# tianhao-stan-wu/LLA-MPC

Hardware: AMD Instinct MI355X
Metric: model-rollouts/sec (N_models x H steps) per control tick; wall-clock per plan() call (higher is better)
Workload: dtype f64

## Files before the change

lla-mpc_amd/csrc/dev_wave.hpp:

```cpp
#pragma once
#include <hip/hip_runtime.h>
#include <stdint.h>

#include "kernels.hpp"

namespace llampc {

namespace {

template <int NAN_FIRST>
__device__ __forceinline__ bool kless(double av, int64_t ai, double bv, int64_t bi) {
  return NAN_FIRST ? less_nan_first(av, ai, bv, bi) : less_nan_last(av, ai, bv, bi);
}

constexpr int kDppXor1 = 0xB1, kDppXor2 = 0x4E, kDppRor4 = 0x124, kDppRor8 = 0x128;
template <int CTRL>
__device__ __forceinline__ int dpp_i(int x) {
  return __builtin_amdgcn_update_dpp(x, x, CTRL, 0xF, 0xF, false);
}
template <int CTRL>
__device__ __forceinline__ double dpp_d(double v) {
  return __hiloint2double(dpp_i<CTRL>(__double2hiint(v)), dpp_i<CTRL>(__double2loint(v)));
}
template <int CTRL>
// ... 119 lines not shown
__device__ __forceinline__ uint64_t join_words(uint64_t hi, uint64_t lo) {
  return ((uint64_t)(uint32_t)hi << 32) | (uint32_t)lo;
}

__device__ __forceinline__ int wave_sum(int x) {
  x += dpp_i<kDppXor1>(x);
  x += dpp_i<kDppXor2>(x);
  x += dpp_i<kDppRor4>(x);
  x += dpp_i<kDppRor8>(x);
  return __builtin_amdgcn_readlane(x, 0) + __builtin_amdgcn_readlane(x, 16) +
         __builtin_amdgcn_readlane(x, 32) + __builtin_amdgcn_readlane(x, 48);
}

__device__ __forceinline__ void pin_vgpr(double& x) { asm volatile("" : "+v"(x)); }

}

constexpr int kScratchBytes = 192;
constexpr int kFlagOff = 160;
constexpr int kLateOff = 168;
constexpr int kStageW = 8;
constexpr int kRankBytes = 64 * 8 + 64 * 4 + 256;
constexpr int kWaves = kBlock / 64;
constexpr int kListsPerLane = 8;

struct Scratch {
  double* sv;
  int64_t* si;
  int32_t* sn;
  __device__ explicit Scratch(unsigned char* smem)
// ... 40 lines not shown
```

lla-mpc_amd/csrc/kernels.hip:

```cpp
#include <stdlib.h>

#include <algorithm>

#include "dev_wave.hpp"
#include "final_dev.hpp"
#include "lookback_dev.hpp"
#include "peer_dev.hpp"
#include "rollout_dev.hpp"

namespace llampc {

__global__ __launch_bounds__(kBlock) void merge_kernel(const llampc_plan_out* parts, int32_t G,
                                                       int32_t nan_first, llampc_plan_out* m) {
  extern __shared__ __attribute__((aligned(16))) unsigned char smem[];
  const int tid = threadIdx.x;
  llampc_plan_out* rec = reinterpret_cast<llampc_plan_out*>(smem);
  constexpr int kWords = sizeof(llampc_plan_out) / 16;
  static_assert(sizeof(llampc_plan_out) % 16 == 0, "records staged as 16-B words");
  const uint4* srcw = reinterpret_cast<const uint4*>(parts);
  uint4* dstw = reinterpret_cast<uint4*>(rec);
  for (int e = tid; e < G * kWords; e += kBlock) dstw[e] = srcw[e];
  __syncthreads();
  merge_staged(rec, G, nan_first, m, reinterpret_cast<EntS*>(smem + (size_t)G * sizeof(llampc_plan_out)), 0);
}
// ... 225 lines not shown
      if (base + rl > kLdsMax) {
        stage = false;
        base = kScratchBytes + 16 * (size_t)(la->H + 1);
      }
      const size_t per_seg = 32 * (size_t)std::max(1, la->rl.M);
      const size_t room = base + rl < kLdsMax ? kLdsMax - base - rl : 0;
      lav.rl.wcap = (int32_t)std::min<size_t>(room / per_seg, (size_t)(la->rl.n - 1));
      lds = std::max(lds, base + rl + per_seg * (size_t)lav.rl.wcap);
    } else {
      lds = std::max(lds, lookahead_lds_bytes(la->C, la->H, &stage));
    }
  }
  f.do_lb = lb != nullptr;
  f.do_la = la != nullptr;
  if (f.nb_lb + f.nb_la == 0) return hipErrorInvalidValue;
  int wq = 0;
  if (la && la->wq && lpm == 1 && G <= 64 && integ == LLAMPC_RK4 && la->xref_mode == LLAMPC_XREF_GIVEN &&
      !pk && getenv("LLAMPC_NO_WQ") == nullptr) {
    const int nw = std::max(1, device_cus() - 1);
    const char* force = getenv("LLAMPC_WQ_WAVES");
    const int forced = force ? atoi(force) : 0;
    if ((int64_t)f.nb_la * 4 >= (int64_t)nw * 7 || (forced && f.nb_la > nw)) {
      const int64_t mpw = 64 / G;
      const int64_t units = (la->n + mpw - 1) / mpw;
      f.nb_la = nw;
      wq = (stage && (forced ? forced == 8 : units >= 4 * (int64_t)nw * kWaves)) ? 2 : 1;
    }
  }
  if (f.px_G) {
    if (pk || integ != LLAMPC_RK4 || (la && la->xref_mode == LLAMPC_XREF_RACELINE) || f.px_G > kPeerFuseMax)
      return hipErrorInvalidValue;
    lds = std::max(lds, 256 + (size_t)f.px_G * (sizeof(llampc_plan_out) + 2 * LLAMPC_KMAX * sizeof(EntS)) +
                            kWaves * sizeof(int));
  }

  if (pk) {
    if (!la || !plan_inline_ok(la->C, la->H, integ, la->xref_mode) || !stage) return hipErrorInvalidValue;
    if (lpm == 4) launch_plan_inline_group<4>(lbv, lav, f, G, cpl, lds, s, *pk);
    else if (lpm == 2) launch_plan_inline_group<2>(lbv, lav, f, G, cpl, lds, s, *pk);
    else launch_plan_inline_group<1>(lbv, lav, f, G, cpl, lds, s, *pk);
    return hipGetLastError();
  }
  switch (integ) {
    case LLAMPC_RK4:
    case LLAMPC_EULER_NLP: {
      const bool rk4 = integ == LLAMPC_RK4;
      const int w = rk4 ? wq : 0;
      if (lpm == 4) (rk4 ? launch_plan_group<0, 4> : launch_plan_group<1, 4>)(lbv, lav, f, G, cpl, stage, lds, s, w);
      else if (lpm == 2) (rk4 ? launch_plan_group<0, 2> : launch_plan_group<1, 2>)(lbv, lav, f, G, cpl, stage, lds, s, w);
      else (rk4 ? launch_plan_group<0, 1> : launch_plan_group<1, 1>)(lbv, lav, f, G, cpl, stage, lds, s, w);
      break;
    }
    case LLAMPC_RK6:
      launch_plan_group<2, 1>(lbv, lav, f, G, cpl, stage, lds, s, 0);
      break;
    default: return hipErrorInvalidValue;
  }
  return hipGetLastError();
}


hipError_t launch_merge(const llampc_plan_out* parts, int32_t G, int32_t nan_first,
                        llampc_plan_out* merged, hipStream_t s) {
  if (G < 1 || G > 32) return hipErrorInvalidValue;
  const size_t M = (size_t)G * LLAMPC_KMAX;
  const size_t lds = (size_t)G * sizeof(llampc_plan_out) + 2 * M * sizeof(EntS);
  allow_lds(merge_kernel);
  hipLaunchKernelGGL(merge_kernel, dim3(1), dim3(kBlock), lds, s, parts, G, nan_first, merged);
  return hipGetLastError();
// ... 46 lines not shown
```

lla-mpc_amd/csrc/kernels.hpp:

```cpp
#pragma once
#include <hip/hip_runtime.h>
#include <stdint.h>

#include "dyn.hpp"
#include "raceline.hpp"
#include "llampc.h"

namespace llampc {

constexpr int kBlock = 256;
constexpr int kBlockWQ = 512;
constexpr int wq_threads(int wq) { return wq == 2 ? kBlockWQ : kBlock; }

struct CostK {
  double Q[4], R[4], P[4];
  double umin[2], umax[2];
  double dmax[2];
  int32_t enforce;
  int32_t pad;
};

struct LookbackLaunch {
  const double* params;  int64_t n;  int64_t goff;
  VehK veh;
// ... 40 lines not shown
  const double* am_val; const int64_t* am_idx; const double* tk_val; const int64_t* tk_idx;
  const double* pv; const int64_t* pidx; const int32_t* pnf;
  const uint64_t* la_tag; const uint64_t* blk_tag;
  uint32_t seq;
  int32_t poll;
  uint64_t* host_tag;
  uint64_t host_seq;
  uint64_t* const* px_box;
  llampc_plan_out* px_merged;
  int32_t px_G, px_rank;
  uint32_t px_seq;
  uint32_t px_bound;
  uint64_t* wq;
};

constexpr int kInlineDoubles = 352;
struct InlinePack {
  double v[kInlineDoubles];
};

int lookback_blocks(int64_t n);
int lookahead_group(int32_t C);
int lookahead_lpm(int64_t n, int32_t C, int32_t integrator, int32_t share = 1);
int lookahead_blocks(int64_t n, int32_t C, int lpm);
int lookback_r(int64_t n, int32_t K);
int lookback_blocks_r(int64_t n, int R);
size_t lookahead_lds_bytes(int32_t C, int32_t H, bool* stage_u);
size_t raceline_lds_bytes(int32_t n, int32_t M);

hipError_t launch_plan(const LookbackLaunch* lb, const LookaheadLaunch* la, FinalLaunch f,
                       hipStream_t s, const InlinePack* pk = nullptr, int32_t share = 1);
bool plan_inline_ok(int32_t C, int32_t H, int32_t integrator, int32_t xref_mode);
template <int INTEG, int LPM>
void launch_plan_group(const LookbackLaunch& lb, const LookaheadLaunch& la, const FinalLaunch& f, int G,
                       int cpl, bool stage, size_t lds, hipStream_t s, int wq);
template <int LPM>
void launch_plan_inline_group(const LookbackLaunch& lb, const LookaheadLaunch& la, const FinalLaunch& f,
                              int G, int cpl, size_t lds, hipStream_t s, const InlinePack& pk);
#define LLAMPC_PLAN_GROUP_DECL(I, L)                                                               \
  extern template void launch_plan_group<I, L>(const LookbackLaunch&, const LookaheadLaunch&,      \
                                               const FinalLaunch&, int, int, bool, size_t,          \
                                               hipStream_t, int)
LLAMPC_PLAN_GROUP_DECL(0, 4);
LLAMPC_PLAN_GROUP_DECL(0, 2);
LLAMPC_PLAN_GROUP_DECL(0, 1);
LLAMPC_PLAN_GROUP_DECL(1, 4);
LLAMPC_PLAN_GROUP_DECL(1, 2);
LLAMPC_PLAN_GROUP_DECL(1, 1);
LLAMPC_PLAN_GROUP_DECL(2, 1);
extern template void launch_plan_inline_group<4>(const LookbackLaunch&, const LookaheadLaunch&, const FinalLaunch&,
                                                 int, int, size_t, hipStream_t, const InlinePack&);
extern template void launch_plan_inline_group<2>(const LookbackLaunch&, const LookaheadLaunch&, const FinalLaunch&,
                                                 int, int, size_t, hipStream_t, const InlinePack&);
extern template void launch_plan_inline_group<1>(const LookbackLaunch&, const LookaheadLaunch&, const FinalLaunch&,
                                                 int, int, size_t, hipStream_t, const InlinePack&);
template <typename KERN>
static void allow_lds(KERN k) {
  static bool done = false;
  if (!done) {
    (void)hipFuncSetAttribute(reinterpret_cast<const void*>(k), hipFuncAttributeMaxDynamicSharedMemorySize,
                              (int)(160 * 1024));
    done = true;
  }
}
hipError_t launch_merge(const llampc_plan_out* parts, int32_t G, int32_t nan_first,
                        llampc_plan_out* merged, hipStream_t s);
constexpr int kPeerMax = 32;
constexpr int kRecWords = (int)(sizeof(llampc_plan_out) / 4);
struct PeerLaunch {
  const llampc_plan_out* local;
// ... 19 lines not shown
```

lla-mpc_amd/csrc/lookahead_dev.hpp:

```cpp
#pragma once
#include "dev_stamps.hpp"
#include "dev_wave.hpp"
#include "raceline.hpp"
#include "rollout_dev.hpp"

namespace llampc {

template <int NW = kWaves>
__device__ __forceinline__ void la_publish(const LookaheadLaunch& a, int blk, const Scratch& sc, int par,
                                           double v, int64_t key, int nf) {
  static_assert(NW == kWaves || NW == 8, "4- or 8-wave blocks");
  wave_pick_nl64(v, key);
  const int nfw = wave_sum(nf);
  double* sv = sc.sv + 4 * par;
  int64_t* si = sc.si + 4 * par;
  if ((threadIdx.x & 63) == 0) {
    sv[threadIdx.x >> 6] = v;
    si[threadIdx.x >> 6] = key;
    sc.sn[threadIdx.x >> 6] = nfw;
  }
  __syncthreads();
  if (threadIdx.x == 0) {
    int nfs = sc.sn[0];
#pragma unroll
// ... 7 lines not shown
      uint64_t* r = a.blk_tag + 5 * (int64_t)blk;
      const uint64_t vb = (uint64_t)__double_as_longlong(v), kb = (uint64_t)key;
      st_wt(&r[0], tag_word(a.seq, (uint32_t)(vb >> 32)));
      st_wt(&r[1], tag_word(a.seq, (uint32_t)vb));
      st_wt(&r[2], tag_word(a.seq, (uint32_t)(kb >> 32)));
      st_wt(&r[3], tag_word(a.seq, (uint32_t)kb));
      st_wt(&r[4], tag_word(a.seq, (uint32_t)nfs));
    } else {
      st_wt(&a.pv[blk], v);
      st_wt(&a.pidx[blk], key);
      st_wt(&a.pnf[blk], nfs);
    }
  }
}

template <int INTEG, bool STAGE, int LPM, int XM, int WQ = 0>
__device__ __forceinline__ void lookahead_block(const LookaheadLaunch& a, int blk, int G, int cpl,
                                                unsigned char* smem, const Scratch& sc) {
  LA_STAMP(blk, 0);
  constexpr int BT = wq_threads(WQ);
  double* sx = reinterpret_cast<double*>(smem + kScratchBytes);
  double* su = sx + 2 * (a.H + 1);
  const int H = a.H, C = a.C;
  const int sub = threadIdx.x % LPM;
  const int cl = threadIdx.x / LPM;
  const int g = cl & (G - 1);
  const int64_t n = (int64_t)blk * (kBlock / (G * LPM)) + cl / G;
  const bool live = n < a.n;
  const int mpb = kBlock / (G * LPM);
  const int soff = (XM && mpb < kBlock) ? mpb : 0;
  Tire t{};
  if (!WQ && live) t = load_tire(a.params, a.n, n);
  double x0[6];
#pragma unroll
  for (int m = 0; m < 6; ++m) x0[m] = a.x0[m];
  double* rl_knots = su + (STAGE ? kStageW * C * H : 0);
  double* rl_xy = rl_knots + a.rl.n + kKnotPad;
  if (XM) {
    const int nk = a.rl.n, nseg = a.rl.n - 1, nxy = 8 * nseg;
    const double* gk = a.rl.knots;
    const double* gmu = a.rl.mus;
    double* rl_mus = rl_xy + nxy;
    copy_lds<4>(rl_knots, nk, [&](int e) { return gk[e]; });
    copy_lds<24>(rl_xy, nxy + a.rl.M, [&](int e) {
      const double* p = e < nxy ? gk + nk + e : gmu + (e - nxy);
      return *p;
    });
    if ((int)threadIdx.x < kKnotPad) rl_knots[nk + threadIdx.x] = __builtin_inf();
    const double s0 = a.xref[0];
    const double L = gk[nseg];
// ... 69 lines not shown
    RL_STAMP(blk, 3);
  } else {
    for (int e = threadIdx.x; e <= H; e += BT) {
      sx[2 * e] = a.xref[e];
      sx[2 * e + 1] = a.xref[(H + 1) + e];
    }
  }
  fm::FmK K0;
  if constexpr (!XM) K0 = fm::FmK::load<kLeanLA && INTEG == 0>();
  if (STAGE) {
    const fm::FmK K = [&] {
      if constexpr (XM) return fm::FmK::load();
      else return K0;
    }();
    const FusedK fq0 = make_fused(a.veh, make_stage<1>(a.veh, Tire{}, 0), a.Ts, scaled_yaw(LPM));
    for (int e = (int)threadIdx.x - soff; e < C * H; e += BT - soff) {
      if (e < 0) break;
      const int c = e / H, k = e - c * H;
      const double dl = a.U[2 * e + 1];
      double sd, cd;
      if (fm::sincos_fast_ok(dl)) fm::sincos_fast(dl, &sd, &cd, K);
      else LL_SINCOS(dl, &sd, &cd);
      double* o = su + kStageW * (k * C + c);
      const double ua = a.U[2 * e];
      const double p0 = k ? a.U[2 * e - 2] : a.uprev[0], p1 = k ? a.U[2 * e - 1] : a.uprev[1];
      const double d0 = ua - p0, d1 = dl - p1;
      if (INTEG == 0) {
        const FusedIn fi = fused_in(fq0, Input{ua, dl, sd, cd});
        o[0] = fi.F0;
        o[1] = fi.F1;
        o[2] = fi.hmsd;
        o[3] = fi.hmcd;
        o[4] = fi.c5a;
        o[5] = dl;
      } else {
        o[0] = ua;
        o[1] = dl;
        o[2] = sd;
        o[3] = cd;
      }
      o[6] = act_term(a.cost, d0, d1);
      o[7] = (!a.cost.enforce || input_feasible(a.cost, ua, dl, d0, d1)) ? 1.0 : 0.0;
    }
  }
  __syncthreads();

  CostK q = a.cost;
  VehK veh = a.veh;
  double Ts = a.Ts;
  for (int m = 0; m < 4; ++m) {
    pin_vgpr(q.Q[m]);
    pin_vgpr(q.R[m]);
    pin_vgpr(q.P[m]);
  }
  for (int m = 0; m < 2; ++m) {
    pin_vgpr(q.umin[m]);
    pin_vgpr(q.umax[m]);
    pin_vgpr(q.dmax[m]);
  }
  pin_vgpr(veh.lf);
  pin_vgpr(veh.lr);
  pin_vgpr(veh.mass);
  pin_vgpr(veh.inv_mass);
  pin_vgpr(veh.inv_Iz);
  pin_vgpr(veh.Cm1);
  pin_vgpr(veh.Cm2);
  pin_vgpr(veh.Cr0);
  pin_vgpr(veh.Cr2);
  pin_vgpr(Ts);
  const double up0 = a.uprev[0], up1 = a.uprev[1];

  double bv = __builtin_nan("");
  int64_t bc = kNoIndex;
  int nf = 0;
  LA_STAMP(blk, 1);
  constexpr bool kSplit = (INTEG == 0 && LPM == 4);
  constexpr unsigned kRF = (STAGE ? kRStage : 0u) | (XM ? kRXm : 0u);
  constexpr unsigned kRSplitQ = kSplit ? kRSplit : 0u;
  const bool diagQP = a.cost.Q[1] == 0.0 && a.cost.Q[2] == 0.0 && a.cost.P[1] == 0.0 && a.cost.P[2] == 0.0;
  if constexpr (WQ) {
    static_assert(LPM == 1 && XM == 0, "work queue: LPM 1, shared xref");
    const int mpw = 64 / G;
    const int64_t units = (a.n + mpw - 1) / mpw;
    const int lm = (int)(threadIdx.x & 63) / G;
    uint32_t zoff;
    asm volatile("v_mov_b32 %0, 0" : "=v"(zoff));
    auto issue = [&](uint32_t off) -> uint64_t {
      uint64_t v = 0;
      if ((threadIdx.x & 63) == 0)
        v = __hip_atomic_fetch_add(a.wq + off, (uint64_t)1, __ATOMIC_RELAXED, __HIP_MEMORY_SCOPE_AGENT);
      return v;
    };
    auto take = [&](uint64_t v) -> int64_t {
      const uint32_t lo = (uint32_t)__builtin_amdgcn_readlane((int)(uint32_t)v, 0);
// ... 184 lines not shown
```

lla-mpc_amd/csrc/plan_dev.hpp:

```cpp
#pragma once
#include <algorithm>

#include "final_dev.hpp"
#include "lookahead_dev.hpp"
#include "lookback_dev.hpp"
#include "peer_dev.hpp"

namespace llampc {

template <int INTEG, bool STAGE, int LPM, int XM, bool PX = false, int WQ = 0>
__device__ __forceinline__ void plan_body(const LookbackLaunch& lb, const LookaheadLaunch& la,
                                          const FinalLaunch& fin, int G, int cpl) {
  extern __shared__ __attribute__((aligned(16))) unsigned char smem[];
  const Scratch sc(smem);
  int* flag = reinterpret_cast<int*>(smem + kFlagOff);
  const bool is_lb = (int)blockIdx.x < fin.nb_lb;
  const int lb_blk = (int)blockIdx.x, la_blk = (int)blockIdx.x - fin.nb_lb;
  if constexpr (wq_threads(WQ) > kBlock) {
    if (is_lb && threadIdx.x >= kBlock) return;
  }
  if (is_lb) {
    lookback_block(lb, lb_blk, sc);
    if (!ticket_last(&fin.tickets[0], (unsigned)fin.nb_lb, flag)) return;
    if (fin.full) {
      lb_final(fin, smem);
      if (fin.host_tag) __threadfence_system();
    }
    if (fin.poll) {
      __syncthreads();
      final_poll(fin, sc);
      if constexpr (PX) peer_finish(fin, smem);
      return;
    }
  } else {
    lookahead_block<INTEG, STAGE, LPM, XM, WQ>(la, la_blk, G, cpl, smem, sc);
    if (fin.poll) return;
    if constexpr (wq_threads(WQ) > kBlock) {
      if (threadIdx.x >= kBlock) return;
    }
  }
  const unsigned expected = (unsigned)fin.nb_la + (fin.nb_lb > 0 ? 1u : 0u);
  if (!ticket_last(&fin.tickets[1], expected, flag)) return;
  final_select(fin, sc);
  if constexpr (PX) peer_finish(fin, smem);
}

template <int INTEG, bool STAGE, int LPM, int XM, bool PX = false, int WQ = 0>
__global__ __launch_bounds__(wq_threads(WQ)) void plan_kernel(LookbackLaunch lb, LookaheadLaunch la,
                                                      FinalLaunch fin, int G, int cpl) {
  plan_body<INTEG, STAGE, LPM, XM, PX, WQ>(lb, la, fin, G, cpl);
}

template <int LPM>
__global__ __launch_bounds__(kBlock) void plan_kernel_inl(LookbackLaunch lb, LookaheadLaunch la,
                                                          FinalLaunch fin, int G, int cpl,
                                                          InlinePack pk) {
  const double* v = pk.v;
  lb.x_prev = v;
  lb.u_prev = v + 6;
  lb.x_now = v + 8;
  la.x0 = v + 8;
  la.uprev = v + 14;
  la.xref = v + 16;
  la.U = v + 16 + 2 * (la.H + 1);
  plan_body<0, true, LPM, 0>(lb, la, fin, G, cpl);
}

constexpr size_t kOneBlockPerCuLds = 82 * 1024;

template <int INTEG, bool STAGE, int PX, int WQ>
static void launch_plan_wq(const LookbackLaunch& lb, const LookaheadLaunch& la, const FinalLaunch& f,
                           int G, int cpl, size_t lds, hipStream_t s) {
  allow_lds(plan_kernel<INTEG, STAGE, 1, 0, PX, WQ>);
  hipLaunchKernelGGL((plan_kernel<INTEG, STAGE, 1, 0, PX, WQ>), dim3(f.nb_lb + f.nb_la), dim3(wq_threads(WQ)),
                     lds, s, lb, la, f, G, cpl);
}

template <int INTEG, bool STAGE, int LPM>
static void launch_plan_t(const LookbackLaunch& lb, const LookaheadLaunch& la, const FinalLaunch& f,
                          int G, int cpl, size_t lds, hipStream_t s, int wq = 0) {
  lds = std::max(lds, kOneBlockPerCuLds);
  if constexpr (INTEG == LLAMPC_RK4 && LPM == 1) {
    if (wq) {
      if constexpr (STAGE) {
        if (wq == 2) {
          if (f.px_G) launch_plan_wq<INTEG, STAGE, 1, 2>(lb, la, f, G, cpl, lds, s);
          else launch_plan_wq<INTEG, STAGE, 0, 2>(lb, la, f, G, cpl, lds, s);
          return;
        }
      }
      if (f.px_G) launch_plan_wq<INTEG, STAGE, 1, 1>(lb, la, f, G, cpl, lds, s);
      else launch_plan_wq<INTEG, STAGE, 0, 1>(lb, la, f, G, cpl, lds, s);
      return;
    }
  }
  if constexpr (INTEG == LLAMPC_RK4) {
    if (f.px_G) {
      allow_lds(plan_kernel<INTEG, STAGE, LPM, 0, true>);
      hipLaunchKernelGGL((plan_kernel<INTEG, STAGE, LPM, 0, true>), dim3(f.nb_lb + f.nb_la), dim3(kBlock), lds,
                         s, lb, la, f, G, cpl);
      return;
    }
  }
  if (la.xref_mode == LLAMPC_XREF_RACELINE) {
    allow_lds(plan_kernel<INTEG, STAGE, LPM, 1>);
    hipLaunchKernelGGL((plan_kernel<INTEG, STAGE, LPM, 1>), dim3(f.nb_lb + f.nb_la), dim3(kBlock), lds, s,
                       lb, la, f, G, cpl);
  } else {
    allow_lds(plan_kernel<INTEG, STAGE, LPM, 0>);
    hipLaunchKernelGGL((plan_kernel<INTEG, STAGE, LPM, 0>), dim3(f.nb_lb + f.nb_la), dim3(kBlock), lds, s,
                       lb, la, f, G, cpl);
  }
}

template <int LPM>
static void launch_plan_inl(const LookbackLaunch& lb, const LookaheadLaunch& la, const FinalLaunch& f,
                            int G, int cpl, size_t lds, hipStream_t s, const InlinePack& pk) {
  lds = std::max(lds, kOneBlockPerCuLds);
  allow_lds(plan_kernel_inl<LPM>);
  hipLaunchKernelGGL((plan_kernel_inl<LPM>), dim3(f.nb_lb + f.nb_la), dim3(kBlock), lds, s, lb, la, f,
                     G, cpl, pk);
}

template <int INTEG, int LPM>
void launch_plan_group(const LookbackLaunch& lb, const LookaheadLaunch& la, const FinalLaunch& f, int G,
                       int cpl, bool stage, size_t lds, hipStream_t s, int wq) {
  if (stage) launch_plan_t<INTEG, true, LPM>(lb, la, f, G, cpl, lds, s, wq);
  else launch_plan_t<INTEG, false, LPM>(lb, la, f, G, cpl, lds, s, wq);
}

template <int LPM>
void launch_plan_inline_group(const LookbackLaunch& lb, const LookaheadLaunch& la, const FinalLaunch& f,
                              int G, int cpl, size_t lds, hipStream_t s, const InlinePack& pk) {
  launch_plan_inl<LPM>(lb, la, f, G, cpl, lds, s, pk);
}

}
```

lla-mpc_amd/csrc/plan_euler.hip:

```cpp
#include "plan_dev.hpp"

namespace llampc {

template void launch_plan_group<1, 4>(const LookbackLaunch&, const LookaheadLaunch&, const FinalLaunch&, int,
                                            int, bool, size_t, hipStream_t, int);
template void launch_plan_group<1, 2>(const LookbackLaunch&, const LookaheadLaunch&, const FinalLaunch&, int,
                                            int, bool, size_t, hipStream_t, int);
template void launch_plan_group<1, 1>(const LookbackLaunch&, const LookaheadLaunch&, const FinalLaunch&, int,
                                            int, bool, size_t, hipStream_t, int);

}
```

lla-mpc_amd/csrc/plan_rk4_l1.hip:

```cpp
#include "plan_dev.hpp"

namespace llampc {

template void launch_plan_group<0, 1>(const LookbackLaunch&, const LookaheadLaunch&, const FinalLaunch&, int,
                                            int, bool, size_t, hipStream_t, int);
template void launch_plan_inline_group<1>(const LookbackLaunch&, const LookaheadLaunch&, const FinalLaunch&,
                                              int, int, size_t, hipStream_t, const InlinePack&);

}

#ifdef LLAMPC_STAMPS
namespace llampc {
extern "C" int llampc_debug_wq_units(unsigned long long* out) {
  return hipMemcpyFromSymbol(out, HIP_SYMBOL(g_wq_unit), sizeof(g_wq_unit)) == hipSuccess ? 0 : -2;
}
extern "C" int llampc_debug_wq_reset() {
  void* p = nullptr;
  if (hipGetSymbolAddress(&p, HIP_SYMBOL(g_wq_unit)) != hipSuccess) return -2;
  return hipMemset(p, 0, sizeof(g_wq_unit)) == hipSuccess ? 0 : -2;
}
}
#endif
```

lla-mpc_amd/csrc/plan_rk4_l2.hip:

```cpp
#include "plan_dev.hpp"

namespace llampc {

template void launch_plan_group<0, 2>(const LookbackLaunch&, const LookaheadLaunch&, const FinalLaunch&, int,
                                            int, bool, size_t, hipStream_t, int);
template void launch_plan_inline_group<2>(const LookbackLaunch&, const LookaheadLaunch&, const FinalLaunch&,
                                              int, int, size_t, hipStream_t, const InlinePack&);

}
```

lla-mpc_amd/csrc/plan_rk4_l4.hip:

```cpp
#include "plan_dev.hpp"

namespace llampc {

template void launch_plan_group<0, 4>(const LookbackLaunch&, const LookaheadLaunch&, const FinalLaunch&, int,
                                            int, bool, size_t, hipStream_t, int);
template void launch_plan_inline_group<4>(const LookbackLaunch&, const LookaheadLaunch&, const FinalLaunch&,
                                              int, int, size_t, hipStream_t, const InlinePack&);

}

#ifdef LLAMPC_STAMPS
namespace llampc {
extern "C" int llampc_debug_lb_stamps(unsigned long long* out) {
  return hipMemcpyFromSymbol(out, HIP_SYMBOL(g_lb_stamps), sizeof(g_lb_stamps)) == hipSuccess ? 0 : -2;
}
extern "C" int llampc_debug_rl_ph(unsigned long long* out) {
  return hipMemcpyFromSymbol(out, HIP_SYMBOL(g_rl_ph), sizeof(g_rl_ph)) == hipSuccess ? 0 : -2;
}
extern "C" int llampc_debug_rl(double* out) {
  return hipMemcpyFromSymbol(out, HIP_SYMBOL(g_rl_dbg), sizeof(g_rl_dbg)) == hipSuccess ? 0 : -2;
}
extern "C" int llampc_debug_la_wave(unsigned long long* out) {
  return hipMemcpyFromSymbol(out, HIP_SYMBOL(g_la_wave), sizeof(g_la_wave)) == hipSuccess ? 0 : -2;
}
// ... 16 lines not shown
```

lla-mpc_amd/csrc/plan_rk6.hip:

```cpp
#include "plan_dev.hpp"

namespace llampc {

template void launch_plan_group<2, 1>(const LookbackLaunch&, const LookaheadLaunch&, const FinalLaunch&, int,
                                            int, bool, size_t, hipStream_t, int);

}
```

Before: 8.347 billion.

## Pack plan kernel arguments into a single head-first kernarg struct with scalar pinning

Replaces the separate lookback/lookahead/final launch structs with one PlanArgs kernarg block. Its leading PlanHead holds the hot shared fields within a few adjacent cache lines, and the role structs are read in 16-byte words. Device code reads fields through kernarg-segment pointers, pins pointers and scalars into SGPRs via readfirstlane and address-space casts, and hoists the initial U/uprev/x0 loads so they overlap LDS staging. The aim is to cut kernel-argument fetch latency and stop the compiler from carrying uniform values in VGPRs. In exchange it adds inline-asm constraints that could hurt scheduling, plus a host-side consistency check on the argument structs.

```diff
diff --git a/lla-mpc_amd/csrc/dev_wave.hpp b/lla-mpc_amd/csrc/dev_wave.hpp
--- a/lla-mpc_amd/csrc/dev_wave.hpp
+++ b/lla-mpc_amd/csrc/dev_wave.hpp
@@ -157,6 +157,32 @@
 
 __device__ __forceinline__ void pin_vgpr(double& x) { asm volatile("" : "+v"(x)); }
 
+template <typename T>
+__device__ __forceinline__ void as_global(T*& p) {
+  auto g = (__attribute__((address_space(1))) T*)p;
+  asm volatile("" : "+s"(g));
+  p = (T*)g;
+}
+
+__device__ __forceinline__ uint32_t lane_zero() {
+  uint32_t z;
+  asm("v_mov_b32 %0, 0" : "=v"(z));
+  return z;
+}
+template <typename T>
+__device__ __forceinline__ T uni(T v) {
+  static_assert(sizeof(T) % 4 == 0, "whole 32-bit words");
+  uint32_t w[sizeof(T) / 4];
+  __builtin_memcpy(w, &v, sizeof(T));
+#pragma unroll
+  for (unsigned i = 0; i < sizeof(T) / 4; ++i) {
+    asm volatile("" : "+v"(w[i]));
+    w[i] = (uint32_t)__builtin_amdgcn_readfirstlane((int)w[i]);
+  }
+  __builtin_memcpy(&v, w, sizeof(T));
+  return v;
+}
+
 }
 
 constexpr int kScratchBytes = 192;
diff --git a/lla-mpc_amd/csrc/kernels.hip b/lla-mpc_amd/csrc/kernels.hip
--- a/lla-mpc_amd/csrc/kernels.hip
+++ b/lla-mpc_amd/csrc/kernels.hip
@@ -263,6 +263,7 @@
   f.do_lb = lb != nullptr;
   f.do_la = la != nullptr;
   if (f.nb_lb + f.nb_la == 0) return hipErrorInvalidValue;
+  if (!plan_args_consistent(lb, la, f)) return hipErrorInvalidValue;
   int wq = 0;
   if (la && la->wq && lpm == 1 && G <= 64 && integ == LLAMPC_RK4 && la->xref_mode == LLAMPC_XREF_GIVEN &&
       !pk && getenv("LLAMPC_NO_WQ") == nullptr) {
@@ -283,11 +284,12 @@
                             kWaves * sizeof(int));
   }
 
+  const PlanArgs a = plan_args(lb ? &lbv : nullptr, la ? &lav : nullptr, f, G, cpl);
   if (pk) {
     if (!la || !plan_inline_ok(la->C, la->H, integ, la->xref_mode) || !stage) return hipErrorInvalidValue;
-    if (lpm == 4) launch_plan_inline_group<4>(lbv, lav, f, G, cpl, lds, s, *pk);
-    else if (lpm == 2) launch_plan_inline_group<2>(lbv, lav, f, G, cpl, lds, s, *pk);
-    else launch_plan_inline_group<1>(lbv, lav, f, G, cpl, lds, s, *pk);
+    if (lpm == 4) launch_plan_inline_group<4>(a, lds, s, *pk);
+    else if (lpm == 2) launch_plan_inline_group<2>(a, lds, s, *pk);
+    else launch_plan_inline_group<1>(a, lds, s, *pk);
     return hipGetLastError();
   }
   switch (integ) {
@@ -295,13 +297,13 @@
     case LLAMPC_EULER_NLP: {
       const bool rk4 = integ == LLAMPC_RK4;
       const int w = rk4 ? wq : 0;
-      if (lpm == 4) (rk4 ? launch_plan_group<0, 4> : launch_plan_group<1, 4>)(lbv, lav, f, G, cpl, stage, lds, s, w);
-      else if (lpm == 2) (rk4 ? launch_plan_group<0, 2> : launch_plan_group<1, 2>)(lbv, lav, f, G, cpl, stage, lds, s, w);
-      else (rk4 ? launch_plan_group<0, 1> : launch_plan_group<1, 1>)(lbv, lav, f, G, cpl, stage, lds, s, w);
+      if (lpm == 4) (rk4 ? launch_plan_group<0, 4> : launch_plan_group<1, 4>)(a, stage, lds, s, w);
+      else if (lpm == 2) (rk4 ? launch_plan_group<0, 2> : launch_plan_group<1, 2>)(a, stage, lds, s, w);
+      else (rk4 ? launch_plan_group<0, 1> : launch_plan_group<1, 1>)(a, stage, lds, s, w);
       break;
     }
     case LLAMPC_RK6:
-      launch_plan_group<2, 1>(lbv, lav, f, G, cpl, stage, lds, s, 0);
+      launch_plan_group<2, 1>(a, stage, lds, s, 0);
       break;
     default: return hipErrorInvalidValue;
   }
diff --git a/lla-mpc_amd/csrc/kernels.hpp b/lla-mpc_amd/csrc/kernels.hpp
--- a/lla-mpc_amd/csrc/kernels.hpp
+++ b/lla-mpc_amd/csrc/kernels.hpp
@@ -1,5 +1,6 @@
 #pragma once
 #include <hip/hip_runtime.h>
+#include <stddef.h>
 #include <stdint.h>
 
 #include "dyn.hpp"
@@ -78,6 +79,72 @@
   uint64_t* wq;
 };
 
+struct PlanHead {
+  int32_t nb_lb;
+  int32_t poll;
+  int64_t n, goff;
+  int32_t C, H, G, cpl;
+  const double* params;
+  const double* x0; const double* U; const double* xref; const double* uprev;
+  uint64_t* la_tag; uint64_t* blk_tag;
+  const double* x_prev; const double* u_prev; const double* x_now;
+  double* ring;
+  int32_t W, slot;
+};
+struct alignas(16) PlanArgs {
+  PlanHead hd;
+  alignas(16) LookaheadLaunch la;
+  alignas(16) LookbackLaunch lb;
+  alignas(16) FinalLaunch fin;
+};
+constexpr size_t kKernargLine = 64;
+static_assert(offsetof(PlanArgs, hd) == 0, "the head leads the kernarg segment");
+static_assert(offsetof(PlanHead, blk_tag) + sizeof(uint64_t*) <= 2 * kKernargLine,
+              "the look-ahead's head: two adjacent lines");
+static_assert(sizeof(PlanHead) <= 3 * kKernargLine, "the whole head: one batch of adjacent lines");
+static_assert(offsetof(PlanArgs, la) % 16 == 0 && offsetof(PlanArgs, lb) % 16 == 0 &&
+                  offsetof(PlanArgs, fin) % 16 == 0 && sizeof(PlanArgs) % 16 == 0,
+              "the role structs are read in 16-byte words");
+
+inline PlanArgs plan_args(const LookbackLaunch* lb, const LookaheadLaunch* la, const FinalLaunch& f, int G,
+                          int cpl) {
+  PlanArgs a{};
+  if (la) a.la = *la;
+  if (lb) a.lb = *lb;
+  a.fin = f;
+  PlanHead& h = a.hd;
+  h.nb_lb = f.nb_lb;
+  h.poll = f.poll;
+  h.n = la ? la->n : lb ? lb->n : f.n;
+  h.goff = la ? la->goff : lb ? lb->goff : f.goff;
+  h.params = la ? la->params : lb ? lb->params : f.params;
+  h.C = a.la.C;
+  h.H = a.la.H;
+  h.G = G;
+  h.cpl = cpl;
+  h.x0 = a.la.x0;
+  h.U = a.la.U;
+  h.xref = a.la.xref;
+  h.uprev = a.la.uprev;
+  h.la_tag = a.la.la_tag;
+  h.blk_tag = a.la.blk_tag;
+  h.x_prev = a.lb.x_prev;
+  h.u_prev = a.lb.u_prev;
+  h.x_now = a.lb.x_now;
+  h.ring = a.lb.ring;
+  h.W = a.lb.W;
+  h.slot = a.lb.slot;
+  return a;
+}
+inline bool plan_args_consistent(const LookbackLaunch* lb, const LookaheadLaunch* la, const FinalLaunch& f) {
+  if (lb && la && (lb->params != la->params || lb->n != la->n || lb->goff != la->goff)) return false;
+  if (la && (la->poll != 0) != (f.poll != 0)) return false;
+  if (la && f.poll && (la->la_tag != f.la_tag || la->blk_tag != f.blk_tag || la->seq != f.seq)) return false;
+  const int64_t n = la ? la->n : lb ? lb->n : f.n, goff = la ? la->goff : lb ? lb->goff : f.goff;
+  const double* params = la ? la->params : lb ? lb->params : f.params;
+  return f.n == n && f.goff == goff && f.params == params;
+}
+
 constexpr int kInlineDoubles = 352;
 struct InlinePack {
   double v[kInlineDoubles];
@@ -96,15 +163,11 @@
                        hipStream_t s, const InlinePack* pk = nullptr, int32_t share = 1);
 bool plan_inline_ok(int32_t C, int32_t H, int32_t integrator, int32_t xref_mode);
 template <int INTEG, int LPM>
-void launch_plan_group(const LookbackLaunch& lb, const LookaheadLaunch& la, const FinalLaunch& f, int G,
-                       int cpl, bool stage, size_t lds, hipStream_t s, int wq);
+void launch_plan_group(const PlanArgs& a, bool stage, size_t lds, hipStream_t s, int wq);
 template <int LPM>
-void launch_plan_inline_group(const LookbackLaunch& lb, const LookaheadLaunch& la, const FinalLaunch& f,
-                              int G, int cpl, size_t lds, hipStream_t s, const InlinePack& pk);
-#define LLAMPC_PLAN_GROUP_DECL(I, L)                                                               \
-  extern template void launch_plan_group<I, L>(const LookbackLaunch&, const LookaheadLaunch&,      \
-                                               const FinalLaunch&, int, int, bool, size_t,          \
-                                               hipStream_t, int)
+void launch_plan_inline_group(const PlanArgs& a, size_t lds, hipStream_t s, const InlinePack& pk);
+#define LLAMPC_PLAN_GROUP_DECL(I, L) \
+  extern template void launch_plan_group<I, L>(const PlanArgs&, bool, size_t, hipStream_t, int)
 LLAMPC_PLAN_GROUP_DECL(0, 4);
 LLAMPC_PLAN_GROUP_DECL(0, 2);
 LLAMPC_PLAN_GROUP_DECL(0, 1);
@@ -112,12 +175,9 @@
 LLAMPC_PLAN_GROUP_DECL(1, 2);
 LLAMPC_PLAN_GROUP_DECL(1, 1);
 LLAMPC_PLAN_GROUP_DECL(2, 1);
-extern template void launch_plan_inline_group<4>(const LookbackLaunch&, const LookaheadLaunch&, const FinalLaunch&,
-                                                 int, int, size_t, hipStream_t, const InlinePack&);
-extern template void launch_plan_inline_group<2>(const LookbackLaunch&, const LookaheadLaunch&, const FinalLaunch&,
-                                                 int, int, size_t, hipStream_t, const InlinePack&);
-extern template void launch_plan_inline_group<1>(const LookbackLaunch&, const LookaheadLaunch&, const FinalLaunch&,
-                                                 int, int, size_t, hipStream_t, const InlinePack&);
+extern template void launch_plan_inline_group<4>(const PlanArgs&, size_t, hipStream_t, const InlinePack&);
+extern template void launch_plan_inline_group<2>(const PlanArgs&, size_t, hipStream_t, const InlinePack&);
+extern template void launch_plan_inline_group<1>(const PlanArgs&, size_t, hipStream_t, const InlinePack&);
 template <typename KERN>
 static void allow_lds(KERN k) {
   static bool done = false;
diff --git a/lla-mpc_amd/csrc/lookahead_dev.hpp b/lla-mpc_amd/csrc/lookahead_dev.hpp
--- a/lla-mpc_amd/csrc/lookahead_dev.hpp
+++ b/lla-mpc_amd/csrc/lookahead_dev.hpp
@@ -45,10 +45,43 @@
   }
 }
 
+__device__ __forceinline__ void la_args_uniform(LookaheadLaunch& a) {
+  a.veh.input_acc = uni(a.veh.input_acc);
+  a.veh.approx = uni(a.veh.approx);
+  a.cost.enforce = uni(a.cost.enforce);
+  a.cost_out = uni(a.cost_out);
+  a.best_cand = uni(a.best_cand);
+  a.best_cost = uni(a.best_cost);
+  a.pv = uni(a.pv);
+  a.pidx = uni(a.pidx);
+  a.pnf = uni(a.pnf);
+  a.seq = uni(a.seq);
+  a.wq = uni(a.wq);
+  as_global(a.cost_out);
+  as_global(a.best_cand);
+  as_global(a.best_cost);
+  as_global(a.pv);
+  as_global(a.pidx);
+  as_global(a.pnf);
+  as_global(a.wq);
+}
+
 template <int INTEG, bool STAGE, int LPM, int XM, int WQ = 0>
-__device__ __forceinline__ void lookahead_block(const LookaheadLaunch& a, int blk, int G, int cpl,
+__device__ __forceinline__ void lookahead_block(const LookaheadLaunch& args, int blk, int G, int cpl,
                                                 unsigned char* smem, const Scratch& sc) {
   LA_STAMP(blk, 0);
+  LookaheadLaunch a = args;
+  if constexpr (XM) {
+    a.rl = uni(a.rl);
+    a.xref_pm = uni(a.xref_pm);
+    as_global(a.rl.knots);
+    as_global(a.rl.xy);
+    as_global(a.rl.speed);
+    as_global(a.rl.mus);
+    as_global(a.xref_pm);
+    a.Ts = uni(a.Ts);
+    a.veh.mass = uni(a.veh.mass);
+  }
   constexpr int BT = wq_threads(WQ);
   double* sx = reinterpret_cast<double*>(smem + kScratchBytes);
   double* su = sx + 2 * (a.H + 1);
@@ -62,9 +95,21 @@
   const int soff = (XM && mpb < kBlock) ? mpb : 0;
   Tire t{};
   if (!WQ && live) t = load_tire(a.params, a.n, n);
+  const uint32_t lz = lane_zero();
   double x0[6];
 #pragma unroll
-  for (int m = 0; m < 6; ++m) x0[m] = a.x0[m];
+  for (int m = 0; m < 6; ++m) x0[m] = a.x0[lz + m];
+  double up0 = a.uprev[lz], up1 = a.uprev[lz + 1];
+  const int e0 = (int)threadIdx.x - soff;
+  double u0a = 0.0, u0d = 0.0, u0pa = 0.0, u0pd = 0.0;
+  if (STAGE && e0 >= 0 && e0 < C * H) {
+    u0a = a.U[2 * e0];
+    u0d = a.U[2 * e0 + 1];
+    if (e0 > 0) {
+      u0pa = a.U[2 * e0 - 2];
+      u0pd = a.U[2 * e0 - 1];
+    }
+  }
   double* rl_knots = su + (STAGE ? kStageW * C * H : 0);
   double* rl_xy = rl_knots + a.rl.n + kKnotPad;
   if (XM) {
@@ -164,16 +209,17 @@
       else return K0;
     }();
     const FusedK fq0 = make_fused(a.veh, make_stage<1>(a.veh, Tire{}, 0), a.Ts, scaled_yaw(LPM));
-    for (int e = (int)threadIdx.x - soff; e < C * H; e += BT - soff) {
+    for (int e = e0; e < C * H; e += BT - soff) {
       if (e < 0) break;
+      const bool first = e == e0;
       const int c = e / H, k = e - c * H;
-      const double dl = a.U[2 * e + 1];
+      const double dl = first ? u0d : a.U[2 * e + 1];
       double sd, cd;
       if (fm::sincos_fast_ok(dl)) fm::sincos_fast(dl, &sd, &cd, K);
       else LL_SINCOS(dl, &sd, &cd);
       double* o = su + kStageW * (k * C + c);
-      const double ua = a.U[2 * e];
-      const double p0 = k ? a.U[2 * e - 2] : a.uprev[0], p1 = k ? a.U[2 * e - 1] : a.uprev[1];
+      const double ua = first ? u0a : a.U[2 * e];
+      const double p0 = !k ? up0 : first ? u0pa : a.U[2 * e - 2], p1 = !k ? up1 : first ? u0pd : a.U[2 * e - 1];
       const double d0 = ua - p0, d1 = dl - p1;
       if (INTEG == 0) {
         const FusedIn fi = fused_in(fq0, Input{ua, dl, sd, cd});
@@ -195,6 +241,7 @@
   }
   __syncthreads();
 
+  la_args_uniform(a);
   CostK q = a.cost;
   VehK veh = a.veh;
   double Ts = a.Ts;
@@ -218,7 +265,10 @@
   pin_vgpr(veh.Cr0);
   pin_vgpr(veh.Cr2);
   pin_vgpr(Ts);
-  const double up0 = a.uprev[0], up1 = a.uprev[1];
+#pragma unroll
+  for (int m = 0; m < 6; ++m) x0[m] = uni(x0[m]);
+  up0 = uni(up0);
+  up1 = uni(up1);
 
   double bv = __builtin_nan("");
   int64_t bc = kNoIndex;
@@ -227,7 +277,8 @@
   constexpr bool kSplit = (INTEG == 0 && LPM == 4);
   constexpr unsigned kRF = (STAGE ? kRStage : 0u) | (XM ? kRXm : 0u);
   constexpr unsigned kRSplitQ = kSplit ? kRSplit : 0u;
-  const bool diagQP = a.cost.Q[1] == 0.0 && a.cost.Q[2] == 0.0 && a.cost.P[1] == 0.0 && a.cost.P[2] == 0.0;
+  const bool diagQP =
+      uni((int)(a.cost.Q[1] == 0.0 && a.cost.Q[2] == 0.0 && a.cost.P[1] == 0.0 && a.cost.P[2] == 0.0)) != 0;
   if constexpr (WQ) {
     static_assert(LPM == 1 && XM == 0, "work queue: LPM 1, shared xref");
     const int mpw = 64 / G;
diff --git a/lla-mpc_amd/csrc/plan_dev.hpp b/lla-mpc_amd/csrc/plan_dev.hpp
--- a/lla-mpc_amd/csrc/plan_dev.hpp
+++ b/lla-mpc_amd/csrc/plan_dev.hpp
@@ -8,131 +8,270 @@
 
 namespace llampc {
 
+typedef uint32_t karg_w4 __attribute__((ext_vector_type(4)));
+#define LLAMPC_KARG __attribute__((address_space(4)))
+__device__ __forceinline__ uint32_t karg_fence(uint32_t off) {
+  asm volatile("" : "+s"(off));
+  return off;
+}
+template <typename T>
+__device__ __forceinline__ T karg_read(uint32_t w16) {
+  constexpr int NW = (int)((sizeof(T) + 15) / 16);
+  const LLAMPC_KARG karg_w4* p =
+      (const LLAMPC_KARG karg_w4*)__builtin_amdgcn_kernarg_segment_ptr() + karg_fence(w16);
+  karg_w4 w[NW];
+#pragma unroll
+  for (int i = 0; i < NW; ++i) w[i] = p[i];
+  T v;
+  __builtin_memcpy(&v, w, sizeof(T));
+  return v;
+}
+template <typename T>
+__device__ __forceinline__ T karg_field(uint32_t off) {
+  const LLAMPC_KARG unsigned char* p =
+      (const LLAMPC_KARG unsigned char*)__builtin_amdgcn_kernarg_segment_ptr() + karg_fence(off);
+  return *reinterpret_cast<const LLAMPC_KARG T*>(p);
+}
+
+template <typename T>
+__device__ __forceinline__ void pin_sgpr(T& x) {
+  asm volatile("" : "+s"(x));
+}
+template <typename T>
+__device__ __forceinline__ void pin_sgpr(T*& p) {
+  as_global(p);
+}
+__device__ __forceinline__ PlanHead head_pinned(PlanHead h) {
+  pin_sgpr(h.nb_lb);
+  pin_sgpr(h.poll);
+  pin_sgpr(h.n);
+  pin_sgpr(h.goff);
+  pin_sgpr(h.C);
+  pin_sgpr(h.H);
+  pin_sgpr(h.G);
+  pin_sgpr(h.cpl);
+  pin_sgpr(h.params);
+  pin_sgpr(h.x0);
+  pin_sgpr(h.U);
+  pin_sgpr(h.xref);
+  pin_sgpr(h.uprev);
+  pin_sgpr(h.la_tag);
+  pin_sgpr(h.blk_tag);
+  pin_sgpr(h.x_prev);
+  pin_sgpr(h.u_prev);
+  pin_sgpr(h.x_now);
+  pin_sgpr(h.ring);
+  pin_sgpr(h.W);
+  pin_sgpr(h.slot);
+  return h;
+}
+
+__device__ __forceinline__ LookaheadLaunch lookahead_args(const PlanHead& hd) {
+  const LookaheadLaunch* p = reinterpret_cast<const LookaheadLaunch*>(
+      (const unsigned char*)__builtin_amdgcn_kernarg_segment_ptr() + offsetof(PlanArgs, la) + 16 * lane_zero());
+  LookaheadLaunch a;
+  a.params = hd.params;
+  a.n = hd.n;
+  a.goff = hd.goff;
+  a.x0 = hd.x0;
+  a.U = hd.U;
+  a.xref = hd.xref;
+  a.uprev = hd.uprev;
+  a.C = hd.C;
+  a.H = hd.H;
+  a.la_tag = hd.la_tag;
+  a.blk_tag = hd.blk_tag;
+  a.poll = hd.poll != 0;
+  a.veh = p->veh;
+  a.integrator = p->integrator;
+  a.Ts = p->Ts;
+  a.cost = p->cost;
+  a.cost_out = p->cost_out;
+  a.best_cand = p->best_cand;
+  a.best_cost = p->best_cost;
+  a.pv = p->pv;
+  a.pidx = p->pidx;
+  a.pnf = p->pnf;
+  a.xref_mode = p->xref_mode;
+  a.rl = p->rl;
+  a.xref_pm = p->xref_pm;
+  a.seq = p->seq;
+  a.wq = p->wq;
+  return a;
+}
+
+__device__ __forceinline__ LookbackLaunch lookback_args(const PlanHead& hd) {
+  LookbackLaunch a = karg_read<LookbackLaunch>((uint32_t)(offsetof(PlanArgs, lb) / 16));
+  a.params = hd.params;
+  a.n = hd.n;
+  a.goff = hd.goff;
+  a.x_prev = hd.x_prev;
+  a.u_prev = hd.u_prev;
+  a.x_now = hd.x_now;
+  a.ring = hd.ring;
+  a.W = hd.W;
+  a.slot = hd.slot;
+  pin_sgpr(a.err_out);
+  pin_sgpr(a.wm_buf);
+  pin_sgpr(a.am_val);
+  pin_sgpr(a.am_idx);
+  pin_sgpr(a.tk_val);
+  pin_sgpr(a.tk_idx);
+  return a;
+}
+
+__device__ __forceinline__ FinalLaunch final_args() {
+  FinalLaunch f = karg_read<FinalLaunch>((uint32_t)(offsetof(PlanArgs, fin) / 16));
+  pin_sgpr(f.out);
+  pin_sgpr(f.tickets);
+  pin_sgpr(f.params);
+  pin_sgpr(f.best_cand);
+  pin_sgpr(f.best_cost);
+  pin_sgpr(f.am_val);
+  pin_sgpr(f.am_idx);
+  pin_sgpr(f.tk_val);
+  pin_sgpr(f.tk_idx);
+  pin_sgpr(f.pv);
+  pin_sgpr(f.pidx);
+  pin_sgpr(f.pnf);
+  pin_sgpr(f.la_tag);
+  pin_sgpr(f.blk_tag);
+  pin_sgpr(f.host_tag);
+  pin_sgpr(f.px_box);
+  pin_sgpr(f.px_merged);
+  pin_sgpr(f.wq);
+  return f;
+}
+__device__ __forceinline__ unsigned* ticket_words() {
+  unsigned* t = karg_field<unsigned*>((uint32_t)(offsetof(PlanArgs, fin) + offsetof(FinalLaunch, tickets)));
+  pin_sgpr(t);
+  return t;
+}
+
 template <int INTEG, bool STAGE, int LPM, int XM, bool PX = false, int WQ = 0>
-__device__ __forceinline__ void plan_body(const LookbackLaunch& lb, const LookaheadLaunch& la,
-                                          const FinalLaunch& fin, int G, int cpl) {
+__device__ __forceinline__ void plan_body(const PlanHead& head) {
+  const PlanHead hd = head_pinned(head);
   extern __shared__ __attribute__((aligned(16))) unsigned char smem[];
   const Scratch sc(smem);
   int* flag = reinterpret_cast<int*>(smem + kFlagOff);
-  const bool is_lb = (int)blockIdx.x < fin.nb_lb;
-  const int lb_blk = (int)blockIdx.x, la_blk = (int)blockIdx.x - fin.nb_lb;
+  const bool is_lb = (int)blockIdx.x < hd.nb_lb;
+  const int lb_blk = (int)blockIdx.x, la_blk = (int)blockIdx.x - hd.nb_lb;
   if constexpr (wq_threads(WQ) > kBlock) {
     if (is_lb && threadIdx.x >= kBlock) return;
   }
+  constexpr uint32_t kNbLaOff = (uint32_t)(offsetof(PlanArgs, fin) + offsetof(FinalLaunch, nb_la));
   if (is_lb) {
+    const LookbackLaunch lb = lookback_args(hd);
     lookback_block(lb, lb_blk, sc);
-    if (!ticket_last(&fin.tickets[0], (unsigned)fin.nb_lb, flag)) return;
+    if (!ticket_last(&ticket_words()[0], (unsigned)hd.nb_lb, flag)) return;
+    const FinalLaunch fin = final_args();
     if (fin.full) {
       lb_final(fin, smem);
       if (fin.host_tag) __threadfence_system();
     }
-    if (fin.poll) {
+    if (hd.poll) {
       __syncthreads();
       final_poll(fin, sc);
       if constexpr (PX) peer_finish(fin, smem);
       return;
     }
   } else {
-    lookahead_block<INTEG, STAGE, LPM, XM, WQ>(la, la_blk, G, cpl, smem, sc);
-    if (fin.poll) return;
+    const LookaheadLaunch la = lookahead_args(hd);
+    lookahead_block<INTEG, STAGE, LPM, XM, WQ>(la, la_blk, hd.G, hd.cpl, smem, sc);
+    if (hd.poll) return;
     if constexpr (wq_threads(WQ) > kBlock) {
       if (threadIdx.x >= kBlock) return;
     }
   }
-  const unsigned expected = (unsigned)fin.nb_la + (fin.nb_lb > 0 ? 1u : 0u);
-  if (!ticket_last(&fin.tickets[1], expected, flag)) return;
+  const unsigned expected = (unsigned)karg_field<int32_t>(kNbLaOff) + (hd.nb_lb > 0 ? 1u : 0u);
+  if (!ticket_last(&ticket_words()[1], expected, flag)) return;
+  const FinalLaunch fin = final_args();
   final_select(fin, sc);
   if constexpr (PX) peer_finish(fin, smem);
 }
 
 template <int INTEG, bool STAGE, int LPM, int XM, bool PX = false, int WQ = 0>
-__global__ __launch_bounds__(wq_threads(WQ)) void plan_kernel(LookbackLaunch lb, LookaheadLaunch la,
-                                                      FinalLaunch fin, int G, int cpl) {
-  plan_body<INTEG, STAGE, LPM, XM, PX, WQ>(lb, la, fin, G, cpl);
+__global__ __launch_bounds__(wq_threads(WQ)) void plan_kernel(PlanArgs args) {
+  plan_body<INTEG, STAGE, LPM, XM, PX, WQ>(args.hd);
 }
 
 template <int LPM>
-__global__ __launch_bounds__(kBlock) void plan_kernel_inl(LookbackLaunch lb, LookaheadLaunch la,
-                                                          FinalLaunch fin, int G, int cpl,
-                                                          InlinePack pk) {
-  const double* v = pk.v;
-  lb.x_prev = v;
-  lb.u_prev = v + 6;
-  lb.x_now = v + 8;
-  la.x0 = v + 8;
-  la.uprev = v + 14;
-  la.xref = v + 16;
-  la.U = v + 16 + 2 * (la.H + 1);
-  plan_body<0, true, LPM, 0>(lb, la, fin, G, cpl);
+__global__ __launch_bounds__(kBlock) void plan_kernel_inl(PlanArgs args, InlinePack pk) {
+  static_assert(sizeof(PlanArgs) + sizeof(InlinePack) <= 4096, "the kernarg segment's limit");
+  PlanHead hd = args.hd;
+  constexpr size_t kPackOff = (sizeof(PlanArgs) + alignof(InlinePack) - 1) / alignof(InlinePack) * alignof(InlinePack);
+  const double* v = reinterpret_cast<const double*>((const unsigned char*)__builtin_amdgcn_kernarg_segment_ptr() + kPackOff);
+  hd.x_prev = v;
+  hd.u_prev = v + 6;
+  hd.x_now = v + 8;
+  hd.x0 = v + 8;
+  hd.uprev = v + 14;
+  hd.xref = v + 16;
+  hd.U = v + 16 + 2 * (hd.H + 1);
+  plan_body<0, true, LPM, 0>(hd);
 }
 
 constexpr size_t kOneBlockPerCuLds = 82 * 1024;
 
 template <int INTEG, bool STAGE, int PX, int WQ>
-static void launch_plan_wq(const LookbackLaunch& lb, const LookaheadLaunch& la, const FinalLaunch& f,
-                           int G, int cpl, size_t lds, hipStream_t s) {
+static void launch_plan_wq(const PlanArgs& a, size_t lds, hipStream_t s) {
   allow_lds(plan_kernel<INTEG, STAGE, 1, 0, PX, WQ>);
-  hipLaunchKernelGGL((plan_kernel<INTEG, STAGE, 1, 0, PX, WQ>), dim3(f.nb_lb + f.nb_la), dim3(wq_threads(WQ)),
-                     lds, s, lb, la, f, G, cpl);
+  hipLaunchKernelGGL((plan_kernel<INTEG, STAGE, 1, 0, PX, WQ>), dim3(a.fin.nb_lb + a.fin.nb_la), dim3(wq_threads(WQ)),
+                     lds, s, a);
 }
 
 template <int INTEG, bool STAGE, int LPM>
-static void launch_plan_t(const LookbackLaunch& lb, const LookaheadLaunch& la, const FinalLaunch& f,
-                          int G, int cpl, size_t lds, hipStream_t s, int wq = 0) {
+static void launch_plan_t(const PlanArgs& a, size_t lds, hipStream_t s, int wq = 0) {
   lds = std::max(lds, kOneBlockPerCuLds);
   if constexpr (INTEG == LLAMPC_RK4 && LPM == 1) {
     if (wq) {
       if constexpr (STAGE) {
         if (wq == 2) {
-          if (f.px_G) launch_plan_wq<INTEG, STAGE, 1, 2>(lb, la, f, G, cpl, lds, s);
-          else launch_plan_wq<INTEG, STAGE, 0, 2>(lb, la, f, G, cpl, lds, s);
+          if (a.fin.px_G) launch_plan_wq<INTEG, STAGE, 1, 2>(a, lds, s);
+          else launch_plan_wq<INTEG, STAGE, 0, 2>(a, lds, s);
           return;
         }
       }
-      if (f.px_G) launch_plan_wq<INTEG, STAGE, 1, 1>(lb, la, f, G, cpl, lds, s);
-      else launch_plan_wq<INTEG, STAGE, 0, 1>(lb, la, f, G, cpl, lds, s);
+      if (a.fin.px_G) launch_plan_wq<INTEG, STAGE, 1, 1>(a, lds, s);
+      else launch_plan_wq<INTEG, STAGE, 0, 1>(a, lds, s);
       return;
     }
   }
   if constexpr (INTEG == LLAMPC_RK4) {
-    if (f.px_G) {
+    if (a.fin.px_G) {
       allow_lds(plan_kernel<INTEG, STAGE, LPM, 0, true>);
-      hipLaunchKernelGGL((plan_kernel<INTEG, STAGE, LPM, 0, true>), dim3(f.nb_lb + f.nb_la), dim3(kBlock), lds,
-                         s, lb, la, f, G, cpl);
+      hipLaunchKernelGGL((plan_kernel<INTEG, STAGE, LPM, 0, true>), dim3(a.fin.nb_lb + a.fin.nb_la), dim3(kBlock), lds,
+                         s, a);
       return;
     }
   }
-  if (la.xref_mode == LLAMPC_XREF_RACELINE) {
+  if (a.la.xref_mode == LLAMPC_XREF_RACELINE) {
     allow_lds(plan_kernel<INTEG, STAGE, LPM, 1>);
-    hipLaunchKernelGGL((plan_kernel<INTEG, STAGE, LPM, 1>), dim3(f.nb_lb + f.nb_la), dim3(kBlock), lds, s,
-                       lb, la, f, G, cpl);
+    hipLaunchKernelGGL((plan_kernel<INTEG, STAGE, LPM, 1>), dim3(a.fin.nb_lb + a.fin.nb_la), dim3(kBlock), lds, s,
+                       a);
   } else {
     allow_lds(plan_kernel<INTEG, STAGE, LPM, 0>);
-    hipLaunchKernelGGL((plan_kernel<INTEG, STAGE, LPM, 0>), dim3(f.nb_lb + f.nb_la), dim3(kBlock), lds, s,
-                       lb, la, f, G, cpl);
+    hipLaunchKernelGGL((plan_kernel<INTEG, STAGE, LPM, 0>), dim3(a.fin.nb_lb + a.fin.nb_la), dim3(kBlock), lds, s,
+                       a);
   }
 }
 
 template <int LPM>
-static void launch_plan_inl(const LookbackLaunch& lb, const LookaheadLaunch& la, const FinalLaunch& f,
-                            int G, int cpl, size_t lds, hipStream_t s, const InlinePack& pk) {
+static void launch_plan_inl(const PlanArgs& a, size_t lds, hipStream_t s, const InlinePack& pk) {
   lds = std::max(lds, kOneBlockPerCuLds);
   allow_lds(plan_kernel_inl<LPM>);
-  hipLaunchKernelGGL((plan_kernel_inl<LPM>), dim3(f.nb_lb + f.nb_la), dim3(kBlock), lds, s, lb, la, f,
-                     G, cpl, pk);
+  hipLaunchKernelGGL((plan_kernel_inl<LPM>), dim3(a.fin.nb_lb + a.fin.nb_la), dim3(kBlock), lds, s, a, pk);
 }
 
 template <int INTEG, int LPM>
-void launch_plan_group(const LookbackLaunch& lb, const LookaheadLaunch& la, const FinalLaunch& f, int G,
-                       int cpl, bool stage, size_t lds, hipStream_t s, int wq) {
-  if (stage) launch_plan_t<INTEG, true, LPM>(lb, la, f, G, cpl, lds, s, wq);
-  else launch_plan_t<INTEG, false, LPM>(lb, la, f, G, cpl, lds, s, wq);
+void launch_plan_group(const PlanArgs& a, bool stage, size_t lds, hipStream_t s, int wq) {
+  if (stage) launch_plan_t<INTEG, true, LPM>(a, lds, s, wq);
+  else launch_plan_t<INTEG, false, LPM>(a, lds, s, wq);
 }
 
 template <int LPM>
-void launch_plan_inline_group(const LookbackLaunch& lb, const LookaheadLaunch& la, const FinalLaunch& f,
-                              int G, int cpl, size_t lds, hipStream_t s, const InlinePack& pk) {
-  launch_plan_inl<LPM>(lb, la, f, G, cpl, lds, s, pk);
-}
-
-}
+void launch_plan_inline_group(const PlanArgs& a, size_t lds, hipStream_t s, const InlinePack& pk) {
+  launch_plan_inl<LPM>(a, lds, s, pk);
+}
+
+}
diff --git a/lla-mpc_amd/csrc/plan_euler.hip b/lla-mpc_amd/csrc/plan_euler.hip
--- a/lla-mpc_amd/csrc/plan_euler.hip
+++ b/lla-mpc_amd/csrc/plan_euler.hip
@@ -2,11 +2,8 @@
 
 namespace llampc {
 
-template void launch_plan_group<1, 4>(const LookbackLaunch&, const LookaheadLaunch&, const FinalLaunch&, int,
-                                            int, bool, size_t, hipStream_t, int);
-template void launch_plan_group<1, 2>(const LookbackLaunch&, const LookaheadLaunch&, const FinalLaunch&, int,
-                                            int, bool, size_t, hipStream_t, int);
-template void launch_plan_group<1, 1>(const LookbackLaunch&, const LookaheadLaunch&, const FinalLaunch&, int,
-                                            int, bool, size_t, hipStream_t, int);
+template void launch_plan_group<1, 4>(const PlanArgs&, bool, size_t, hipStream_t, int);
+template void launch_plan_group<1, 2>(const PlanArgs&, bool, size_t, hipStream_t, int);
+template void launch_plan_group<1, 1>(const PlanArgs&, bool, size_t, hipStream_t, int);
 
 }
diff --git a/lla-mpc_amd/csrc/plan_rk4_l1.hip b/lla-mpc_amd/csrc/plan_rk4_l1.hip
--- a/lla-mpc_amd/csrc/plan_rk4_l1.hip
+++ b/lla-mpc_amd/csrc/plan_rk4_l1.hip
@@ -2,10 +2,8 @@
 
 namespace llampc {
 
-template void launch_plan_group<0, 1>(const LookbackLaunch&, const LookaheadLaunch&, const FinalLaunch&, int,
-                                            int, bool, size_t, hipStream_t, int);
-template void launch_plan_inline_group<1>(const LookbackLaunch&, const LookaheadLaunch&, const FinalLaunch&,
-                                              int, int, size_t, hipStream_t, const InlinePack&);
+template void launch_plan_group<0, 1>(const PlanArgs&, bool, size_t, hipStream_t, int);
+template void launch_plan_inline_group<1>(const PlanArgs&, size_t, hipStream_t, const InlinePack&);
 
 }
 
diff --git a/lla-mpc_amd/csrc/plan_rk4_l2.hip b/lla-mpc_amd/csrc/plan_rk4_l2.hip
--- a/lla-mpc_amd/csrc/plan_rk4_l2.hip
+++ b/lla-mpc_amd/csrc/plan_rk4_l2.hip
@@ -2,9 +2,7 @@
 
 namespace llampc {
 
-template void launch_plan_group<0, 2>(const LookbackLaunch&, const LookaheadLaunch&, const FinalLaunch&, int,
-                                            int, bool, size_t, hipStream_t, int);
-template void launch_plan_inline_group<2>(const LookbackLaunch&, const LookaheadLaunch&, const FinalLaunch&,
-                                              int, int, size_t, hipStream_t, const InlinePack&);
+template void launch_plan_group<0, 2>(const PlanArgs&, bool, size_t, hipStream_t, int);
+template void launch_plan_inline_group<2>(const PlanArgs&, size_t, hipStream_t, const InlinePack&);
 
 }
diff --git a/lla-mpc_amd/csrc/plan_rk4_l4.hip b/lla-mpc_amd/csrc/plan_rk4_l4.hip
--- a/lla-mpc_amd/csrc/plan_rk4_l4.hip
+++ b/lla-mpc_amd/csrc/plan_rk4_l4.hip
@@ -2,10 +2,8 @@
 
 namespace llampc {
 
-template void launch_plan_group<0, 4>(const LookbackLaunch&, const LookaheadLaunch&, const FinalLaunch&, int,
-                                            int, bool, size_t, hipStream_t, int);
-template void launch_plan_inline_group<4>(const LookbackLaunch&, const LookaheadLaunch&, const FinalLaunch&,
-                                              int, int, size_t, hipStream_t, const InlinePack&);
+template void launch_plan_group<0, 4>(const PlanArgs&, bool, size_t, hipStream_t, int);
+template void launch_plan_inline_group<4>(const PlanArgs&, size_t, hipStream_t, const InlinePack&);
 
 }
 
diff --git a/lla-mpc_amd/csrc/plan_rk6.hip b/lla-mpc_amd/csrc/plan_rk6.hip
--- a/lla-mpc_amd/csrc/plan_rk6.hip
+++ b/lla-mpc_amd/csrc/plan_rk6.hip
@@ -2,7 +2,6 @@
 
 namespace llampc {
 
-template void launch_plan_group<2, 1>(const LookbackLaunch&, const LookaheadLaunch&, const FinalLaunch&, int,
-                                            int, bool, size_t, hipStream_t, int);
+template void launch_plan_group<2, 1>(const PlanArgs&, bool, size_t, hipStream_t, int);
 
 }
```

Result: no change. 8.335 billion (-0.2%).
